# kirilllzaitsev/vision_mtl

Measured on AMD Instinct MI355X. Metric: images/sec fwd+bwd, basic model 128x256, higher is better.
Workload: dtype f32

## Files before the change

vision_mtl_amd/csrc/conv_pw.hip:

```cpp
#include "common.h"

typedef __bf16 bf16x4 __attribute__((ext_vector_type(4)));
typedef unsigned u32x4 __attribute__((ext_vector_type(4)));
__device__ __forceinline__ u32x2 pw_round_bf16x4(f32x4 v) {
  return __builtin_bit_cast(u32x2, __builtin_convertvector(v, bf16x4));
}
__device__ __forceinline__ bf16x8 pw_round_bf16x8(f32x4 lo, f32x4 hi) {
  const u32x2 l = pw_round_bf16x4(lo), h = pw_round_bf16x4(hi);
  return __builtin_bit_cast(bf16x8, (u32x4){l[0], l[1], h[0], h[1]});
}

struct PwP {
  const float* x;
  const float* wp;
  const float* bias;
  float* y;
  float* stats;
  int M, Ks, ldy, Nw, Cout;
  int tiles_m, tiles_n;
  const float* x2;
  float* y2;
  int K1, N1;
  const float* pa;
  const float* pc;
  const float* res;
  float* a_out;
  int act_in;
  const float* ez_x;
  const float* ez_mean;
  const float* ez_invstd;
  const float* ez_gamma;
  const float* ez_beta;
  const float* ez_add;
  int ez_act;
};

template <int TN, int KW, bool SRC2 = false, bool PRO = false, bool BF16 = false>
__global__ __launch_bounds__(256) void pw_gemm_kernel(PwP p) {
  constexpr int TM = 2;
  constexpr int RG = 4 / KW;
  constexpr int BM = RG * 32;
  constexpr int BN = 16 * TN;
  constexpr int OS = BN + 4;
  __shared__ __attribute__((aligned(16))) float tile[KW][BM][OS];
  __shared__ f32x4 red[2][256];

  const int tid = threadIdx.x, lane = tid & 63, wv = tid >> 6;
  const int l15 = lane & 15, lq = lane >> 4;
  const int ks = wv % KW, rg = wv / KW;
  const int bid = xcd_remap(blockIdx.x, p.tiles_m * p.tiles_n);
  const int tile_m = bid / p.tiles_n, tile_n = bid - tile_m * p.tiles_n;
  const int m0 = tile_m * BM, n0 = tile_n * BN;

  const float* ap[TM];
  const float* ap2[TM];
  const float* bp[TN];
  bool aok[TM], bok[TN];
  const int lda = SRC2 ? p.K1 : p.Ks;
#pragma unroll
  for (int i = 0; i < TM; ++i) {
    const int m = m0 + rg * 32 + 16 * i + l15;
    aok[i] = m < p.M;
    ap[i] = p.x + (size_t)(aok[i] ? m : 0) * lda + 4 * lq;
    ap2[i] = SRC2 ? p.x2 + (size_t)(aok[i] ? m : 0) * (p.Ks - p.K1) + 4 * lq - p.K1 : nullptr;
  }
#pragma unroll
  for (int j = 0; j < TN; ++j) {
    const int n = n0 + 16 * j + l15;
    bok[j] = n < p.Nw;
    bp[j] = p.wp + (size_t)(bok[j] ? n : 0) * p.Ks + 4 * lq;
  }
  const int G = (p.Ks + 15) >> 4;
  f32x4 acc[TM][TN];
#pragma unroll
  for (int i = 0; i < TM; ++i)
#pragma unroll
    for (int j = 0; j < TN; ++j) acc[i][j] = (f32x4){0.f, 0.f, 0.f, 0.f};

  struct Frag { f32x4 a[TM], b[TN], pa, pc, r[TM]; };
  auto load = [&](int g, Frag& f) {
    const bool kok = g < G && 16 * g + 4 * lq < p.Ks;
    if (PRO) {
      f.pa = kok ? *reinterpret_cast<const f32x4*>(p.pa + 16 * g + 4 * lq) : (f32x4){0.f, 0.f, 0.f, 0.f};
      f.pc = kok ? *reinterpret_cast<const f32x4*>(p.pc + 16 * g + 4 * lq) : (f32x4){0.f, 0.f, 0.f, 0.f};
    }
#pragma unroll
    for (int i = 0; i < TM; ++i) {
      const float* src = (SRC2 && 16 * g + 4 * lq >= p.K1) ? ap2[i] : ap[i];
      f.a[i] = (kok && aok[i]) ? *reinterpret_cast<const f32x4*>(src + 16 * g) : (f32x4){0.f, 0.f, 0.f, 0.f};
      if (PRO)
        f.r[i] = (p.res != nullptr && kok && aok[i]) ? *reinterpret_cast<const f32x4*>(p.res + (ap[i] - p.x) + 16 * g)
                                                     : (f32x4){0.f, 0.f, 0.f, 0.f};
    }
#pragma unroll
    for (int j = 0; j < TN; ++j)
      f.b[j] = (kok && bok[j]) ? *reinterpret_cast<const f32x4*>(bp[j] + 16 * g) : (f32x4){0.f, 0.f, 0.f, 0.f};
  };
  auto prologue = [&](Frag& f, int g) {
    if (PRO) {
#pragma unroll
      for (int i = 0; i < TM; ++i) {
        f32x4 v = f.a[i] * f.pa + f.pc;
#pragma unroll
        for (int e = 0; e < 4; ++e) v[e] = act_fwd(v[e], p.act_in);
        v += f.r[i];
        f.a[i] = v;
        if (p.a_out != nullptr && tile_n == 0 && aok[i] && g < G && 16 * g + 4 * lq < p.Ks)
          *reinterpret_cast<f32x4*>(p.a_out + (size_t)(m0 + rg * 32 + 16 * i + l15) * p.Ks + 16 * g + 4 * lq) = v;
      }
    }
  };
  auto mma = [&](Frag& f, int g) {
    prologue(f, g);
#pragma unroll
    for (int e = 0; e < 4; ++e)
#pragma unroll
      for (int i = 0; i < TM; ++i)
#pragma unroll
        for (int j = 0; j < TN; ++j)
          acc[i][j] = __builtin_amdgcn_mfma_f32_16x16x4f32(f.a[i][e], f.b[j][e], acc[i][j], 0, 0, 0);
  };
  if constexpr (!BF16) {
    Frag f0, f1, f2;
    int g = ks;
    load(g, f0);
    load(g + KW, f1);
    for (; g < G; g += 3 * KW) {
      load(g + 2 * KW, f2);
      mma(f0, g);
      if (g + KW >= G) break;
      load(g + 3 * KW, f0);
      mma(f1, g + KW);
      if (g + 2 * KW >= G) break;
      load(g + 4 * KW, f1);
      mma(f2, g + 2 * KW);
    }
  } else {
    constexpr int S = 2 * KW;
    auto load2 = [&](int g, Frag* f) {
      load(g, f[0]);
      load(g + KW, f[1]);
    };
    auto mma2 = [&](Frag* f, int g) {
      prologue(f[0], g);
      prologue(f[1], g + KW);
      bf16x8 fa[TM], fb[TN];
#pragma unroll
      for (int i = 0; i < TM; ++i) fa[i] = pw_round_bf16x8(f[0].a[i], f[1].a[i]);
#pragma unroll
      for (int j = 0; j < TN; ++j) fb[j] = pw_round_bf16x8(f[0].b[j], f[1].b[j]);
#pragma unroll
      for (int i = 0; i < TM; ++i)
#pragma unroll
        for (int j = 0; j < TN; ++j) acc[i][j] = __builtin_amdgcn_mfma_f32_16x16x32_bf16(fa[i], fb[j], acc[i][j], 0, 0, 0);
    };
    Frag f0[2], f1[2];
    int g = ks;
    load2(g, f0);
    for (; g < G; g += 2 * S) {
      load2(g + S, f1);
      mma2(f0, g);
      if (g + S >= G) break;
      load2(g + 2 * S, f0);
      mma2(f1, g + S);
    }
    (void)mma;
  }

#pragma unroll
  for (int i = 0; i < TM; ++i)
#pragma unroll
    for (int j = 0; j < TN; ++j)
#pragma unroll
      for (int r = 0; r < 4; ++r) tile[ks][rg * 32 + 16 * i + 4 * lq + r][16 * j + l15] = acc[i][j][r];
  __syncthreads();

  constexpr int Q = BN / 4;
  constexpr int RPP = 256 / Q;
  constexpr int PASSES = (BM + RPP - 1) / RPP;
  const int q = tid % Q, r0 = tid / Q;
  const int n4 = n0 + 4 * q;
  f32x4 bias4 = {0.f, 0.f, 0.f, 0.f};
  if (p.bias != nullptr) {
#pragma unroll
    for (int e = 0; e < 4; ++e)
      if (n4 + e < p.Nw) bias4[e] = p.bias[n4 + e];
  }
  f32x4 val[PASSES];
  f32x4 s1 = {0.f, 0.f, 0.f, 0.f};
  f32x4 s2x = {0.f, 0.f, 0.f, 0.f};
  const bool ez = p.ez_x != nullptr;
  f32x4 e_mean = {0.f, 0.f, 0.f, 0.f}, e_is = e_mean, e_g = e_mean, e_b = e_mean;
  if (ez && n4 < p.ldy) {
    e_mean = *reinterpret_cast<const f32x4*>(p.ez_mean + n4);
    e_is = *reinterpret_cast<const f32x4*>(p.ez_invstd + n4);
#pragma unroll
    for (int e = 0; e < 4; ++e) {
      e_g[e] = n4 + e < p.Cout ? (p.ez_gamma ? p.ez_gamma[n4 + e] : 1.f) : 0.f;
      e_b[e] = n4 + e < p.Cout ? (p.ez_beta ? p.ez_beta[n4 + e] : 0.f) : 0.f;
    }
  }
  int cnt = 0;
#pragma unroll
  for (int ps = 0; ps < PASSES; ++ps) {
    const int r = r0 + ps * RPP;
    f32x4 v = {0.f, 0.f, 0.f, 0.f};
    if (r < BM) {
      v = *reinterpret_cast<const f32x4*>(&tile[0][r][4 * q]);
#pragma unroll
      for (int k = 1; k < KW; ++k) v += *reinterpret_cast<const f32x4*>(&tile[k][r][4 * q]);
      v += bias4;
#pragma unroll
      for (int e = 0; e < 4; ++e)
        if (n4 + e >= p.Cout) v[e] = 0.f;
      const int m = m0 + r;
      if (ez && m < p.M && n4 < p.ldy) {
        if (p.ez_add != nullptr) v += *reinterpret_cast<const f32x4*>(p.ez_add + (size_t)m * p.ldy + n4);
        const f32x4 xh = (*reinterpret_cast<const f32x4*>(p.ez_x + (size_t)m * p.ldy + n4) - e_mean) * e_is;
        const f32x4 z = e_g * xh + e_b;
#pragma unroll
        for (int e = 0; e < 4; ++e) v[e] *= act_grad(z[e], p.ez_act);
        s2x += v * xh;
      }
      if (m < p.M) {
        if (n4 < p.ldy) {
          if (p.y2 == nullptr) *reinterpret_cast<f32x4*>(p.y + (size_t)m * p.ldy + n4) = v;
          else if (n4 < p.N1) *reinterpret_cast<f32x4*>(p.y + (size_t)m * p.N1 + n4) = v;
          else *reinterpret_cast<f32x4*>(p.y2 + (size_t)m * (p.ldy - p.N1) + (n4 - p.N1)) = v;
        }
        s1 += v;
        ++cnt;
      } else {
        v = (f32x4){0.f, 0.f, 0.f, 0.f};
      }
    }
    val[ps] = v;
  }
  if (p.stats != nullptr && ez) {
    red[0][tid] = s1;
    red[1][tid] = s2x;
    __syncthreads();
// ... 428 lines not shown
  if (variant == 0 && pw_big_cfg(M, ldy, Ks, &c)) {
    const int tiles_m = cdiv(M, c.bm), nprog = pw_big_nprog(M, ldy, c);
    return (M % c.bm == 0 && tiles_m % nprog == 0) ? (tiles_m / nprog) * c.bm : c.bm;
  }
  int tn, kw;
  pw_pick(M, ldy, Ks, &tn, &kw);
  return (4 / kw) * 32;
}

extern "C" int vmtl_conv1x1_stats_rows(int M, int ldy, int Ks, int variant) {
  return cdiv(M, vmtl_conv1x1_stats_block(M, ldy, Ks, variant));
}

static int pw_num_cus() {
  static int n = 0;
  if (n == 0) {
    int dev = 0;
    hipDeviceProp_t prop;
    n = (hipGetDevice(&dev) == hipSuccess && hipGetDeviceProperties(&prop, dev) == hipSuccess && prop.multiProcessorCount > 0)
            ? prop.multiProcessorCount
            : 256;
  }
  return n;
}

template <int TM, int TN, int WM, int WN, int KC, bool BF16>
static int launch_pw_big_t(PwP& p, hipStream_t st) {
  constexpr int BM = WM * TM * 16, BN = WN * TN * 16;
  constexpr int KF = BF16 ? 16 : 32;
  constexpr int A_FLOATS = KC * BM * KF, O_FLOATS = BM * (BN + 4);
  constexpr int NTHR = WM * WN * 64;
  constexpr size_t lds = ((size_t)KC * BN * KF + (A_FLOATS > O_FLOATS ? A_FLOATS : O_FLOATS)) * 4 + 2 * NTHR * 16;
  static_assert(lds <= 160 * 1024, "LDS budget");
  p.tiles_m = cdiv(p.M, BM);
  p.tiles_n = cdiv(p.ldy, BN);
  const BigCfg cfg = {0, BM, BN, KC};
  const int nprog = pw_big_nprog(p.M, p.ldy, cfg);
  const dim3 grid(nprog, p.tiles_n);
#define VMTL_PW_BIG_LAUNCH(SRC2, PRO, EZ)                                                                               \
  {                                                                                                                     \
    static bool attr_set = false;                                                                                       \
    if (!attr_set) {                                                                                                    \
      (void)hipFuncSetAttribute(reinterpret_cast<const void*>(&pw_big_kernel<TM, TN, WM, WN, KC, SRC2, PRO, EZ, BF16>), \
                                hipFuncAttributeMaxDynamicSharedMemorySize, (int)lds);                                 \
      attr_set = true;                                                                                                  \
    }                                                                                                                   \
    hipLaunchKernelGGL((pw_big_kernel<TM, TN, WM, WN, KC, SRC2, PRO, EZ, BF16>), grid, dim3(NTHR), lds, st, p, nprog);  \
  }
  if (p.ez_x != nullptr) VMTL_PW_BIG_LAUNCH(false, false, true)
  else if (p.x2 != nullptr) VMTL_PW_BIG_LAUNCH(true, false, false)
  else if (p.pa != nullptr) VMTL_PW_BIG_LAUNCH(false, true, false)
  else VMTL_PW_BIG_LAUNCH(false, false, false)
#undef VMTL_PW_BIG_LAUNCH
  return vmtl_check_launch();
}

template <int TM, int TN, int WM, int WN, int KC>
static int launch_pw_big(PwP& p, int prec, hipStream_t st) {
  return prec == VMTL_PREC_BF16 ? launch_pw_big_t<TM, TN, WM, WN, KC, true>(p, st)
                                : launch_pw_big_t<TM, TN, WM, WN, KC, false>(p, st);
}

static int pw_big_dispatch(PwP& p, const BigCfg& c, int prec, hipStream_t st) {
  static EnvInt e_w8{"VMTL_PW_BIG_WAVES", 8};
  const bool w8 = env_int(e_w8) == 8;
  switch (c.id) {
    case 0:
      if (w8)
        return c.kc == 2 ? launch_pw_big<2, 2, 2, 4, 2>(p, prec, st) : c.kc == 4 ? launch_pw_big<2, 2, 2, 4, 4>(p, prec, st)
                                                                          : launch_pw_big<2, 2, 2, 4, 6>(p, prec, st);
      return c.kc == 2 ? launch_pw_big<2, 4, 2, 2, 2>(p, prec, st) : c.kc == 4 ? launch_pw_big<2, 4, 2, 2, 4>(p, prec, st)
                                                                        : launch_pw_big<2, 4, 2, 2, 6>(p, prec, st);
    case 1:
      if (w8) return c.kc == 4 ? launch_pw_big<2, 1, 2, 4, 4>(p, prec, st) : launch_pw_big<2, 1, 2, 4, 8>(p, prec, st);
      return c.kc == 4 ? launch_pw_big<2, 2, 2, 2, 4>(p, prec, st) : launch_pw_big<2, 2, 2, 2, 8>(p, prec, st);
    case 2:
      return launch_pw_big<1, 1, 4, 2, 4>(p, prec, st);
    default:
      if (w8) return launch_pw_big<1, 3, 4, 2, 4>(p, prec, st);
      return launch_pw_big<2, 3, 2, 2, 4>(p, prec, st);
  }
}

template <int TN, int KW, bool BF16>
static int launch_pw_t(PwP& p, hipStream_t st) {
  p.tiles_m = cdiv(p.M, (4 / KW) * 32);
  p.tiles_n = cdiv(p.ldy, 16 * TN);
  if (p.x2 != nullptr)
    hipLaunchKernelGGL((pw_gemm_kernel<TN, KW, true, false, BF16>), dim3(p.tiles_m * p.tiles_n), dim3(256), 0, st, p);
  else if (p.pa != nullptr)
    hipLaunchKernelGGL((pw_gemm_kernel<TN, KW, false, true, BF16>), dim3(p.tiles_m * p.tiles_n), dim3(256), 0, st, p);
  else
    hipLaunchKernelGGL((pw_gemm_kernel<TN, KW, false, false, BF16>), dim3(p.tiles_m * p.tiles_n), dim3(256), 0, st, p);
  return vmtl_check_launch();
}

template <int TN, int KW>
static int launch_pw(PwP& p, int prec, hipStream_t st) {
  return prec == VMTL_PREC_BF16 ? launch_pw_t<TN, KW, true>(p, st) : launch_pw_t<TN, KW, false>(p, st);
}

static void pw_plain(PwP& p) {
  p.pa = p.pc = p.res = nullptr; p.a_out = nullptr; p.act_in = 0;
  p.ez_x = p.ez_mean = p.ez_invstd = p.ez_gamma = p.ez_beta = p.ez_add = nullptr; p.ez_act = 0;
}

static int pw_dispatch(PwP& p, int prec, hipStream_t st) {
  BigCfg c;
  if (p.ez_add == nullptr && p.res == nullptr && pw_big_cfg(p.M, p.ldy, p.Ks, &c)) return pw_big_dispatch(p, c, prec, st);
  int tn, kw;
  pw_pick(p.M, p.ldy, p.Ks, &tn, &kw);
  if (tn == 2) return kw == 4 ? launch_pw<2, 4>(p, prec, st) : launch_pw<2, 1>(p, prec, st);
  return kw == 4 ? launch_pw<4, 4>(p, prec, st) : launch_pw<4, 1>(p, prec, st);
}

extern "C" int vmtl_conv1x1_fwd_p(const float* x, const float* wp, const float* bias, float* y, float* stats, int M, int Ks,
                                  int ldy, int Nw, int Cout, int precision, void* stream) {
  VMTL_ENTER();
  if (!valid_prec(precision)) return VMTL_ERR_ARG;
  if (!x || !wp || !y || M <= 0 || Ks <= 0 || (Ks & 3) || ldy <= 0 || (ldy & 3)) return VMTL_ERR_ARG;
  if (Nw <= 0 || Nw > ldy || Cout <= 0 || Cout > Nw) return VMTL_ERR_ARG;
  PwP p;
  p.x = x; p.wp = wp; p.bias = bias; p.y = y; p.stats = stats; p.M = M; p.Ks = Ks; p.ldy = ldy; p.Nw = Nw; p.Cout = Cout;
  p.x2 = nullptr; p.y2 = nullptr; p.K1 = 0; p.N1 = 0;
  pw_plain(p);
  return pw_dispatch(p, precision, (hipStream_t)stream);
}

extern "C" int vmtl_conv1x1_fwd(const float* x, const float* wp, const float* bias, float* y, float* stats, int M, int Ks,
                                int ldy, int Nw, int Cout, void* stream) {
  return vmtl_conv1x1_fwd_p(x, wp, bias, y, stats, M, Ks, ldy, Nw, Cout, VMTL_PREC_FP32, stream);
}

extern "C" int vmtl_conv1x1_cat_fwd_p(const float* x, int K1, const float* x2, int K2s, const float* wp, const float* bias,
                                      float* y, float* stats, int M, int ldy, int Nw, int Cout, int precision,
                                      void* stream) {
  VMTL_ENTER();
  if (!valid_prec(precision)) return VMTL_ERR_ARG;
  if (!x || !x2 || !wp || !y || M <= 0 || K1 <= 0 || (K1 & 3) || K2s <= 0 || (K2s & 3) || ldy <= 0 || (ldy & 3))
    return VMTL_ERR_ARG;
  if (Nw <= 0 || Nw > ldy || Cout <= 0 || Cout > Nw) return VMTL_ERR_ARG;
  PwP p;
  p.x = x; p.wp = wp; p.bias = bias; p.y = y; p.stats = stats; p.M = M; p.Ks = K1 + K2s; p.ldy = ldy; p.Nw = Nw;
  p.Cout = Cout; p.x2 = x2; p.y2 = nullptr; p.K1 = K1; p.N1 = 0;
  pw_plain(p);
  return pw_dispatch(p, precision, (hipStream_t)stream);
}

extern "C" int vmtl_conv1x1_cat_fwd(const float* x, int K1, const float* x2, int K2s, const float* wp, const float* bias,
                                    float* y, float* stats, int M, int ldy, int Nw, int Cout, void* stream) {
  return vmtl_conv1x1_cat_fwd_p(x, K1, x2, K2s, wp, bias, y, stats, M, ldy, Nw, Cout, VMTL_PREC_FP32, stream);
}

extern "C" int vmtl_conv1x1_cat_dgrad_p(const float* dy, const float* wp, float* dx, int N1, float* dx2, int N2s, int N2,
                                        int M, int Ks, int precision, void* stream) {
  VMTL_ENTER();
  if (!valid_prec(precision)) return VMTL_ERR_ARG;
  if (!dy || !wp || !dx || !dx2 || M <= 0 || Ks <= 0 || (Ks & 3) || N1 <= 0 || (N1 & 3) || N2s <= 0 || (N2s & 3) ||
      N2 <= 0 || N2 > N2s)
    return VMTL_ERR_ARG;
  PwP p;
  p.x = dy; p.wp = wp; p.bias = nullptr; p.y = dx; p.stats = nullptr; p.M = M; p.Ks = Ks; p.ldy = N1 + N2s;
  p.Nw = N1 + N2; p.Cout = N1 + N2; p.x2 = nullptr; p.y2 = dx2; p.K1 = 0; p.N1 = N1;
  pw_plain(p);
  return pw_dispatch(p, precision, (hipStream_t)stream);
}

extern "C" int vmtl_conv1x1_cat_dgrad(const float* dy, const float* wp, float* dx, int N1, float* dx2, int N2s, int N2,
                                      int M, int Ks, void* stream) {
  return vmtl_conv1x1_cat_dgrad_p(dy, wp, dx, N1, dx2, N2s, N2, M, Ks, VMTL_PREC_FP32, stream);
}

static int conv1x1_bn_fwd_impl(const float* x, const float* coef_a, const float* coef_c, int act_in, const float* res,
                               float* a_out, const float* wp, const float* bias, float* y, float* stats, int M, int Ks,
                               int ldy, int Nw, int Cout, int prec, void* stream) {
  if (!x || !coef_a || !coef_c || !wp || !y || M <= 0 || Ks <= 0 || (Ks & 3) || ldy <= 0 || (ldy & 3)) return VMTL_ERR_ARG;
  if (Nw <= 0 || Nw > ldy || Cout <= 0 || Cout > Nw) return VMTL_ERR_ARG;
  if (act_in != VMTL_ACT_NONE && act_in != VMTL_ACT_RELU && act_in != VMTL_ACT_HSWISH) return VMTL_ERR_ARG;
  PwP p;
  p.x = x; p.wp = wp; p.bias = bias; p.y = y; p.stats = stats; p.M = M; p.Ks = Ks; p.ldy = ldy; p.Nw = Nw; p.Cout = Cout;
  p.x2 = nullptr; p.y2 = nullptr; p.K1 = 0; p.N1 = 0;
  pw_plain(p);
// ... 92 lines not shown
```

vision_mtl_amd/csrc/conv_wgrad.hip:

```cpp
#include <mutex>
#include <unordered_map>

#include "common.h"

struct WgradP {
  const float* x;
  const float* dy;
  float* slabs;
  int B, H, W, Cs;
  int Ho, Wo, ldy;
  int Nw;
  int KH, KW, stride, pad;
  int Ktot, M;
  int chunk;
  int tiles_kk, tiles_co, splits;
  const float* x2;
  int K1;
};

#define BP 32

typedef __bf16 bf16x2 __attribute__((ext_vector_type(2)));
typedef unsigned u32x4 __attribute__((ext_vector_type(4)));
__device__ __forceinline__ unsigned rne_bf16x2(float lo, float hi) {
  return __builtin_bit_cast(unsigned, __builtin_convertvector((f32x2){lo, hi}, bf16x2));
}
#define WG_BNK 128

__host__ __device__ constexpr int wg_ld(int w, int pm = 1) {
  return pm == 0 ? w + 4 : pm == 1 ? ((w + 47) / 64) * 64 + 16 : ((w + 15) / 32) * 32 + 16;
}
static_assert(wg_ld(16) == 16 && wg_ld(20) == 80 && wg_ld(144) == 144 && wg_ld(128) == 144 && wg_ld(68) == 80 &&
              wg_ld(80) == 80 && wg_ld(84) == 144 && wg_ld(36, 2) == 48 && wg_ld(128, 2) == 144, "wg_ld");

template <int TM, int NTR = 0, int PM = 1, int PD = (TM <= 2 ? 3 : (TM <= 4 && NTR == 0) ? 2 : 1), bool FAST = false,
          bool BF16 = false>
__global__ __launch_bounds__(256) void conv_wgrad_kernel(WgradP p) {
  constexpr int TN = 2;
  constexpr int BMM = TM * 16;
  constexpr int BMC = BMM + NTR;
  constexpr int LDY = wg_ld(BMC, PM);
  constexpr int LDX = wg_ld(WG_BNK, PM);
  constexpr int YQ = BMC / 4;
  constexpr int YIT = (BP * YQ + 255) / 256;
  constexpr int XQ = WG_BNK / 4;
  constexpr int XROWS = 256 / XQ;
  constexpr int XP = BP / XROWS;

  extern __shared__ __attribute__((aligned(16))) float smem[];
  float* Ys = smem;
  float* Xs = smem + 2 * BP * LDY;

  const int tid = threadIdx.x;
  const int lane = tid & 63, wn = tid >> 6;
  const int l15 = lane & 15, lq = lane >> 4;

  const int tiles = p.tiles_kk * p.tiles_co;
  const int bid = xcd_remap(blockIdx.x, tiles * p.splits);
  const int zsl = bid / tiles, trem = bid - zsl * tiles;
  const int kk0 = (trem % p.tiles_kk) * WG_BNK;
  const int co0 = (trem / p.tiles_kk) * BMC;
  const int p_begin = zsl * p.chunk;
  const int p_end = min(p.M, p_begin + p.chunk);

  const int xq = tid % XQ, xr = tid / XQ;
  const int kk = kk0 + xq * 4;
  const bool xok = kk < p.Ktot;
  const int tap = xok ? kk / p.Cs : 0;
  const int ci = kk - tap * p.Cs;
  const int dh = tap / p.KW - p.pad;
  const int dw = tap % p.KW - p.pad;
  const int hw = p.Ho * p.Wo;
  const bool two = p.x2 != nullptr;
  const float* xsrc = two ? (ci < p.K1 ? p.x + ci : p.x2 + (ci - p.K1)) : nullptr;
  const int xstride = two ? (ci < p.K1 ? p.K1 : p.Cs - p.K1) : 0;

  int xb[XP], xho[XP], xwo[XP];
  if (!FAST) {
#pragma unroll
    for (int i = 0; i < XP; ++i) {
      const int m = p_begin + xr + XROWS * i;
      const int b = m / hw;
      const int rem = m - b * hw;
      xb[i] = b;
      xho[i] = rem / p.Wo;
      xwo[i] = rem - xho[i] * p.Wo;
    }
  }
  int s_b = 0, s_ho = 0, s_wo = 0;
  int tw[XP];
  int toff[XP];
  int tyoff[YIT];
  if (FAST) {
    s_b = p_begin / hw;
    const int rem = p_begin - s_b * hw;
    s_ho = rem / p.Wo;
    s_wo = rem - s_ho * p.Wo;
#pragma unroll
    for (int i = 0; i < XP; ++i) {
      tw[i] = (xr + XROWS * i) * p.stride + dw;
      toff[i] = ((dh * p.W + tw[i]) * p.Cs + ci) * 4;
    }
#pragma unroll
    for (int it = 0; it < YIT; ++it) {
      const int idx = tid + it * 256;
      const int row = idx / YQ, q = idx - row * YQ;
      tyoff[it] = (idx < BP * YQ && co0 + q * 4 < p.ldy) ? (row * p.ldy + co0 + q * 4) * 4 : -1;
    }
  }

  f32x4 ry[PD][YIT], rx[PD][XP];
  const __amdgpu_buffer_rsrc_t rs_dy =
      __builtin_amdgcn_make_buffer_rsrc((void*)p.dy, 0, (int)((unsigned)p.M * p.ldy * 4u), 0x00020000);
  const __amdgpu_buffer_rsrc_t rs_x =
      __builtin_amdgcn_make_buffer_rsrc((void*)p.x, 0, (int)((unsigned)p.B * p.H * p.W * p.Cs * 4u), 0x00020000);
  constexpr unsigned OOB = 0xFFFFFFFFu;
  auto bload = [](__amdgpu_buffer_rsrc_t r, unsigned off) -> f32x4 {
    return __builtin_bit_cast(f32x4, __builtin_amdgcn_raw_buffer_load_b128(r, off, 0, 0));
  };
  auto load_tile = [&](int pp, f32x4* ry_s, f32x4* rx_s) {
    if (FAST) {
      const unsigned ybase = (unsigned)pp * (unsigned)p.ldy * 4u;
#pragma unroll
      for (int it = 0; it < YIT; ++it) ry_s[it] = bload(rs_dy, tyoff[it] >= 0 ? ybase + (unsigned)tyoff[it] : OOB);
      const int hin = s_ho * p.stride;
      const int win = s_wo * p.stride;
      const unsigned xbase = (unsigned)((s_b * p.H + hin) * p.W + win) * (unsigned)p.Cs * 4u;
      const bool hok = xok & ((unsigned)(hin + dh) < (unsigned)p.H);
#pragma unroll
      for (int i = 0; i < XP; ++i) {
        const bool ok = hok & ((unsigned)(win + tw[i]) < (unsigned)p.W);
        rx_s[i] = bload(rs_x, ok ? xbase + (unsigned)toff[i] : OOB);
      }
      s_wo += BP;
      if (s_wo >= p.Wo) {
        s_wo = 0;
        if (++s_ho == p.Ho) {
          s_ho = 0;
          ++s_b;
        }
      }
      return;
    }
#pragma unroll
    for (int it = 0; it < YIT; ++it) {
      const int idx = tid + it * 256;
      const int row = idx / YQ, q = idx - row * YQ;
      const int m = pp + row, co = co0 + q * 4;
      const bool ok = idx < BP * YQ && m < p_end && co < p.ldy;
      ry_s[it] = bload(rs_dy, ok ? ((unsigned)m * (unsigned)p.ldy + (unsigned)co) * 4u : OOB);
    }
#pragma unroll
    for (int i = 0; i < XP; ++i) {
      const int m = pp + xr + XROWS * i;
      const int h = xho[i] * p.stride + dh, w = xwo[i] * p.stride + dw;
      const bool ok = xok && m < p_end && (unsigned)h < (unsigned)p.H && (unsigned)w < (unsigned)p.W;
      const unsigned off = ((unsigned)((xb[i] * p.H + h) * p.W + w) * (unsigned)p.Cs + (unsigned)ci) * 4u;
      f32x4 v;
      if (two) {
        v = (f32x4){0.f, 0.f, 0.f, 0.f};
        if (ok) v = *reinterpret_cast<const f32x4*>(xsrc + (size_t)((xb[i] * p.H + h) * p.W + w) * xstride);
      } else {
        v = bload(rs_x, ok ? off : OOB);
      }
      rx_s[i] = v;
      xwo[i] += BP;
      while (xwo[i] >= p.Wo) {
        xwo[i] -= p.Wo;
        if (++xho[i] == p.Ho) {
          xho[i] = 0;
          ++xb[i];
        }
      }
    }
  };
  auto store_tile = [&](int buf, const f32x4* ry_s, const f32x4* rx_s) {
    float* ys = Ys + buf * BP * LDY;
    float* xs = Xs + buf * BP * LDX;
#pragma unroll
    for (int it = 0; it < YIT; ++it) {
      const int idx = tid + it * 256;
      const int row = idx / YQ, q = idx - row * YQ;
      if (idx < BP * YQ) *reinterpret_cast<f32x4*>(ys + row * LDY + q * 4) = ry_s[it];
    }
#pragma unroll
    for (int i = 0; i < XP; ++i) *reinterpret_cast<f32x4*>(xs + (xr + XROWS * i) * LDX + xq * 4) = rx_s[i];
  };

  f32x4 acc[TM][TN];
#pragma unroll
  for (int i = 0; i < TM; ++i)
#pragma unroll
    for (int j = 0; j < TN; ++j) acc[i][j] = (f32x4){0.f, 0.f, 0.f, 0.f};
  float tacc[NTR > 0 ? NTR : 1][TN];
#pragma unroll
  for (int t = 0; t < (NTR > 0 ? NTR : 1); ++t)
#pragma unroll
    for (int j = 0; j < TN; ++j) tacc[t][j] = 0.f;

  const int ntr = NTR > 0 ? max(0, min(NTR, p.Nw - (co0 + BMM))) : 0;
#pragma unroll
  for (int d = 0; d < PD; ++d)
    if (p_begin + d * BP < p_end) load_tile(p_begin + d * BP, ry[d], rx[d]);
  if (p_begin < p_end) store_tile(0, ry[0], rx[0]);
  __syncthreads();
  int cur = 0;
  const int nj = min(TN, max(0, (p.Ktot - (kk0 + wn * TN * 16) + 15) >> 4));
  auto compute = [&](int cb) {
    if (nj == 0) return;
    const float* ys = Ys + cb * BP * LDY + lq * LDY + l15;
    const float* xs = Xs + cb * BP * LDX + lq * LDX + wn * TN * 16 + l15;
    if constexpr (BF16) {
      unsigned fa[TM][4], fb[TN][4];
#pragma unroll
      for (int w = 0; w < 4; ++w) {
#pragma unroll
        for (int i = 0; i < TM; ++i)
          fa[i][w] = rne_bf16x2(ys[8 * w * LDY + i * 16], ys[(8 * w + 4) * LDY + i * 16]);
#pragma unroll
        for (int j = 0; j < TN; ++j)
          fb[j][w] = rne_bf16x2(xs[8 * w * LDX + j * 16], xs[(8 * w + 4) * LDX + j * 16]);
      }
#pragma unroll
      for (int j = 0; j < TN; ++j) {
        if (j > 0 && j >= nj) break;
        const bf16x8 b = __builtin_bit_cast(bf16x8, (u32x4){fb[j][0], fb[j][1], fb[j][2], fb[j][3]});
#pragma unroll
        for (int i = 0; i < TM; ++i)
          acc[i][j] = __builtin_amdgcn_mfma_f32_16x16x32_bf16(
              __builtin_bit_cast(bf16x8, (u32x4){fa[i][0], fa[i][1], fa[i][2], fa[i][3]}), b, acc[i][j], 0, 0, 0);
      }
      if (NTR > 0) {
#pragma unroll
        for (int s = 0; s < BP / 4; ++s) {
          const f32x4 ty = *reinterpret_cast<const f32x4*>(Ys + cb * BP * LDY + (4 * s + lq) * LDY + BMM);
#pragma unroll
          for (int t = 0; t < NTR; ++t) {
            if (t >= ntr) break;
            const float tyr = (float)(__bf16)ty[t];
#pragma unroll
            for (int j = 0; j < TN; ++j)
              tacc[t][j] += tyr * __uint_as_float((s & 1) ? (fb[j][s >> 1] & 0xFFFF0000u) : (fb[j][s >> 1] << 16));
          }
        }
      }
      return;
    }
#pragma unroll
    for (int s = 0; s < BP / 4; ++s) {
      float fa[TM], fb[TN];
#pragma unroll
      for (int i = 0; i < TM; ++i) fa[i] = ys[4 * s * LDY + i * 16];
#pragma unroll
      for (int j = 0; j < TN; ++j) fb[j] = xs[4 * s * LDX + j * 16];
#ifdef VMTL_SETPRIO
      __builtin_amdgcn_s_setprio(1);
#endif
#pragma unroll
      for (int j = 0; j < TN; ++j) {
        if (j > 0 && j >= nj) break;
#pragma unroll
        for (int i = 0; i < TM; ++i) acc[i][j] = __builtin_amdgcn_mfma_f32_16x16x4f32(fa[i], fb[j], acc[i][j], 0, 0, 0);
      }
#ifdef VMTL_SETPRIO
      __builtin_amdgcn_s_setprio(0);
#endif
      if (NTR > 0) {
        const f32x4 ty = *reinterpret_cast<const f32x4*>(Ys + cb * BP * LDY + (4 * s + lq) * LDY + BMM);
#pragma unroll
        for (int t = 0; t < NTR; ++t) {
          if (t >= ntr) break;
#pragma unroll
          for (int j = 0; j < TN; ++j) tacc[t][j] += ty[t] * fb[j];
        }
      }
    }
  };
  for (int base = p_begin; base < p_end; base += PD * BP) {
#pragma unroll
    for (int k = 0; k < PD; ++k) {
      const int pp = base + k * BP;
      if (pp < p_end) {
        if (pp + PD * BP < p_end) load_tile(pp + PD * BP, ry[k], rx[k]);
        compute(cur);
        if (pp + BP < p_end) store_tile(cur ^ 1, ry[(k + 1) % PD], rx[(k + 1) % PD]);
        __syncthreads();
        cur ^= 1;
      }
    }
  }

  float* slab = p.slabs + (size_t)zsl * p.Nw * p.Ktot;
#pragma unroll
  for (int i = 0; i < TM; ++i)
#pragma unroll
    for (int j = 0; j < TN; ++j) {
      const int col = kk0 + (wn * TN + j) * 16 + l15;
#pragma unroll
      for (int r = 0; r < 4; ++r) {
        const int row = co0 + i * 16 + 4 * lq + r;
        if (row < p.Nw && col < p.Ktot) slab[(size_t)row * p.Ktot + col] = acc[i][j][r];
      }
    }
  if (NTR > 0) {
#pragma unroll
    for (int t = 0; t < NTR; ++t)
#pragma unroll
      for (int j = 0; j < TN; ++j) {
        const float v = quarter_sum(tacc[t][j]);
        const int row = co0 + BMM + t;
        const int col = kk0 + (wn * TN + j) * 16 + l15;
        if (lq == 0 && row < p.Nw && col < p.Ktot) slab[(size_t)row * p.Ktot + col] = v;
      }
  }
}

static int wgrad_rows(int Nw) {
  static const int cands[] = {16, 32, 48, 64, 80, 144, 20, 36, 68, 128};
  static const float eff[] = {0.35f, 0.55f, 0.72f, 0.82f, 0.88f, 1.0f, 0.43f, 0.61f, 0.86f, 0.97f};
  constexpr int NC = 10;
  static EnvInt force{"VMTL_FORCE_WG_ROWS", 0};
  if (const int v = env_int(force)) {
    for (int i = 0; i < NC; ++i)
      if (cands[i] == v) return v;
  }
  int best = 16;
  float bc = -1.f;
  for (int i = 0; i < NC; ++i) {
    const float cost = (float)((long long)cdiv(Nw, cands[i]) * cands[i]) / eff[i];
    if (bc < 0.f || cost < bc) {
      best = cands[i];
      bc = cost;
    }
  }
  return best;
}

static int wgrad_lds_bytes(int rows) {
  auto lds = [&](int pm) { return 2 * BP * (wg_ld(rows, pm) + wg_ld(WG_BNK, pm)) * 4; };
  const int base = 160 * 1024 / lds(0);
  if (160 * 1024 / lds(1) >= base) return lds(1);
  if (160 * 1024 / lds(2) >= base) return lds(2);
  return lds(0);
}

static int wgrad_splits_uncached(int M, int Nw, int Ktot);

extern "C" int vmtl_conv2d_wgrad_splits(int M, int Nw, int Ktot) {
  if (M <= 0 || Nw <= 0 || Ktot <= 0) return 0;
  static std::mutex mu;
  static std::unordered_map<unsigned long long, int> memo;
  static int memo_epoch = 0;
  const unsigned long long key = ((unsigned long long)M << 32) ^ ((unsigned long long)Nw << 20) ^ (unsigned long long)Ktot;
  std::lock_guard<std::mutex> lk(mu);
  if (memo_epoch != vmtl_env_epoch) {
    memo.clear();
    memo_epoch = vmtl_env_epoch;
  }
  auto it = memo.find(key);
  if (it != memo.end()) return it->second;
  const int v = wgrad_splits_uncached(M, Nw, Ktot);
  memo.emplace(key, v);
  return v;
}

static int wgrad_splits_uncached(int M, int Nw, int Ktot) {
  const long long tiles = (long long)cdiv(Ktot, WG_BNK) * cdiv(Nw, wgrad_rows(Nw));
  static EnvInt e_steps{"VMTL_WG_MIN_STEPS", 4}, e_small{"VMTL_WG_SMALL_M", 16384}, e_splits{"VMTL_FORCE_WG_SPLITS", 0};
  const int min_steps = env_int(e_steps) < 1 ? 1 : env_int(e_steps), small_m = env_int(e_small);
  const long long max_by_rows = cdiv(M, (M <= small_m ? min_steps : 16) * BP);
  const long long max_by_mem = (32ll << 20) / ((long long)Nw * Ktot);
  long long smax = max_by_rows < max_by_mem ? max_by_rows : max_by_mem;
  if (smax < 1) smax = 1;
  if (const long long v = env_int(e_splits)) {
    if (v >= 1 && v <= max_by_rows) {
      const int chunk = cdiv(cdiv(M, (int)v), BP) * BP;
      return cdiv(M, chunk);
    }
  }
  const int rows = wgrad_rows(Nw);
  int occ = 160 * 1024 / wgrad_lds_bytes(rows);
  if (occ > 4) occ = 4;
  if (rows >= 128 && occ > 2) occ = 2;
  const long long slots = 256ll * occ;
  const double t_pix = (rows / 16.0) * occ * 0.0095;
  const double t_slab = (double)Nw * Ktot * 4.0 / 3.0e6;
  long long best = 1;
  double best_cost = -1.0;
  for (long long sp = 1; sp <= smax; ++sp) {
    const int chunk = cdiv(cdiv(M, (int)sp), BP) * BP;
    const long long nsl = cdiv(M, chunk);
    if (nsl != sp && sp != 1) continue;
    const long long rounds = cdivll(tiles * nsl, slots);
    const double cost = rounds * (chunk + 64.0) * t_pix + nsl * t_slab;
    if (best_cost < 0.0 || cost < best_cost) {
      best = nsl;
      best_cost = cost;
    }
  }
  return (int)best;
}

template <int TM, int NTR, int PM, bool FAST, bool BF16 = false>
static int launch_wgrad_pm(WgradP& p, int splits, hipStream_t st);

template <int BMC>
constexpr int wg_pm() {
  constexpr int base = 160 * 1024 / (2 * BP * (wg_ld(BMC, 0) + wg_ld(WG_BNK, 0)) * 4);
  return 160 * 1024 / (2 * BP * (wg_ld(BMC, 1) + wg_ld(WG_BNK, 1)) * 4) >= base   ? 1
         : 160 * 1024 / (2 * BP * (wg_ld(BMC, 2) + wg_ld(WG_BNK, 2)) * 4) >= base ? 2
                                                                                    : 0;
}
static_assert(wg_pm<144>() == 1 && wg_pm<80>() == 1 && wg_pm<36>() == 2 && wg_pm<68>() == 0 && wg_pm<20>() == 0 &&
                  wg_pm<128>() == 1,
              "wg_pm");

static bool wgrad_fast_ok(const WgradP& p) {
  static EnvInt e{"VMTL_WG_FAST", 1};
  return env_int(e) != 0 && p.x2 == nullptr && p.Wo % BP == 0 && p.chunk % BP == 0;
}

template <int TM, int NTR = 0>
static int launch_wgrad(WgradP& p, int splits, hipStream_t st, int prec) {
  constexpr int PMD = wg_pm<TM * 16 + NTR>();
#ifdef VMTL_TUNING
  static EnvInt e_pad{"VMTL_WG_PAD", -1};
  switch (prec == VMTL_PREC_FP32 ? env_int(e_pad) : -1) {
    case 0: return launch_wgrad_pm<TM, NTR, 0, false>(p, splits, st);
    case 1: return launch_wgrad_pm<TM, NTR, 1, false>(p, splits, st);
    case 2: return launch_wgrad_pm<TM, NTR, 2, false>(p, splits, st);
    default: break;
  }
#endif
  if (p.KH == 1 && p.KW == 1 && p.stride == 1 && p.pad == 0 && p.x2 == nullptr && p.M % BP == 0) {
    p.B = 1; p.H = 1; p.W = p.M; p.Ho = 1; p.Wo = p.M;
  }
  if (prec == VMTL_PREC_BF16) {
    if (wgrad_fast_ok(p)) return launch_wgrad_pm<TM, NTR, PMD, true, true>(p, splits, st);
    return launch_wgrad_pm<TM, NTR, PMD, false, true>(p, splits, st);
  }
  if (wgrad_fast_ok(p)) return launch_wgrad_pm<TM, NTR, PMD, true>(p, splits, st);
  return launch_wgrad_pm<TM, NTR, PMD, false>(p, splits, st);
}

template <int TM, int NTR, int PM, bool FAST, bool BF16>
static int launch_wgrad_pm(WgradP& p, int splits, hipStream_t st) {
  constexpr int BMC = TM * 16 + NTR;
  constexpr int PD = (TM <= 2 ? 3 : (TM <= 4 && NTR == 0) ? 2 : 1);
  const size_t lds = (size_t)2 * BP * (wg_ld(BMC, PM) + wg_ld(WG_BNK, PM)) * sizeof(float);
  static bool attr_set = false;
  if (!attr_set) {
    (void)hipFuncSetAttribute(reinterpret_cast<const void*>(&conv_wgrad_kernel<TM, NTR, PM, PD, FAST, BF16>),
                              hipFuncAttributeMaxDynamicSharedMemorySize, (int)lds);
    attr_set = true;
  }
  if ((long long)p.M * p.ldy * 4 >= (1ll << 32) || (long long)p.B * p.H * p.W * p.Cs * 4 >= (1ll << 32))
    return VMTL_ERR_UNSUPPORTED;
  p.tiles_kk = cdiv(p.Ktot, WG_BNK);
  p.tiles_co = cdiv(p.Nw, BMC);
  p.splits = splits;
  hipLaunchKernelGGL((conv_wgrad_kernel<TM, NTR, PM, PD, FAST, BF16>), dim3(p.tiles_kk * p.tiles_co * splits), dim3(256), lds, st,
                     p);
  return vmtl_check_launch();
}

static int wgrad_dispatch(WgradP& p, int splits, void* stream, int prec);

extern "C" int vmtl_conv2d_wgrad_p(const float* x, const float* dy, float* slabs, int splits, int B, int H, int W,
                                   int Cs, int Ho, int Wo, int ldy, int Nw, int KH, int KW, int stride, int pad,
                                   int precision, void* stream) {
  VMTL_ENTER();
  if (!valid_prec(precision) || !x || !dy || !slabs) return VMTL_ERR_ARG;
  if (Cs <= 0 || (Cs & 3) || (ldy & 3) || Nw <= 0 || Nw > ldy) return VMTL_ERR_ARG;
  if ((H + 2 * pad - KH) / stride + 1 != Ho || (W + 2 * pad - KW) / stride + 1 != Wo) return VMTL_ERR_ARG;
  if ((long long)B * Ho * Wo > 0x7fffffffLL || (long long)B * H * W > 0x7fffffffLL) return VMTL_ERR_ARG;
  WgradP p;
  p.x = x; p.dy = dy; p.slabs = slabs; p.B = B; p.H = H; p.W = W; p.Cs = Cs; p.Ho = Ho; p.Wo = Wo; p.ldy = ldy;
  p.Nw = Nw; p.KH = KH; p.KW = KW; p.stride = stride; p.pad = pad; p.Ktot = KH * KW * Cs; p.M = B * Ho * Wo;
  p.x2 = nullptr; p.K1 = 0;
  return wgrad_dispatch(p, splits, stream, precision);
}

extern "C" int vmtl_conv2d_wgrad(const float* x, const float* dy, float* slabs, int splits, int B, int H, int W,
                                 int Cs, int Ho, int Wo, int ldy, int Nw, int KH, int KW, int stride, int pad,
                                 void* stream) {
  return vmtl_conv2d_wgrad_p(x, dy, slabs, splits, B, H, W, Cs, Ho, Wo, ldy, Nw, KH, KW, stride, pad, VMTL_PREC_FP32,
                             stream);
}

extern "C" int vmtl_conv1x1_cat_wgrad_p(const float* x, int K1, const float* x2, int K2s, const float* dy, float* slabs,
                                        int splits, int M, int ldy, int Nw, int precision, void* stream) {
  VMTL_ENTER();
  if (!valid_prec(precision)) return VMTL_ERR_ARG;
  if (!x || !x2 || !dy || !slabs || M <= 0 || K1 <= 0 || (K1 & 3) || K2s <= 0 || (K2s & 3) || (ldy & 3) || Nw <= 0 ||
      Nw > ldy)
    return VMTL_ERR_ARG;
  WgradP p;
  p.x = x; p.dy = dy; p.slabs = slabs; p.B = 1; p.H = 1; p.W = M; p.Cs = K1 + K2s; p.Ho = 1; p.Wo = M; p.ldy = ldy;
  p.Nw = Nw; p.KH = 1; p.KW = 1; p.stride = 1; p.pad = 0; p.Ktot = p.Cs; p.M = M;
  p.x2 = x2; p.K1 = K1;
  return wgrad_dispatch(p, splits, stream, precision);
}

extern "C" int vmtl_conv1x1_cat_wgrad(const float* x, int K1, const float* x2, int K2s, const float* dy, float* slabs,
                                      int splits, int M, int ldy, int Nw, void* stream) {
  return vmtl_conv1x1_cat_wgrad_p(x, K1, x2, K2s, dy, slabs, splits, M, ldy, Nw, VMTL_PREC_FP32, stream);
}

static int wgrad_dispatch(WgradP& p, int splits, void* stream, int prec) {
  const int Nw = p.Nw;
  if (splits != vmtl_conv2d_wgrad_splits(p.M, Nw, p.Ktot)) return VMTL_ERR_ARG;
  p.chunk = cdiv(cdiv(p.M, splits), BP) * BP;
  hipStream_t st = (hipStream_t)stream;
  switch (wgrad_rows(Nw)) {
    case 16: return launch_wgrad<1>(p, splits, st, prec);
    case 32: return launch_wgrad<2>(p, splits, st, prec);
    case 48: return launch_wgrad<3>(p, splits, st, prec);
    case 64: return launch_wgrad<4>(p, splits, st, prec);
    case 80: return launch_wgrad<5>(p, splits, st, prec);
    case 20: return launch_wgrad<1, 4>(p, splits, st, prec);
    case 36: return launch_wgrad<2, 4>(p, splits, st, prec);
    case 68: return launch_wgrad<4, 4>(p, splits, st, prec);
    case 128: return launch_wgrad<8>(p, splits, st, prec);
    default: return launch_wgrad<9>(p, splits, st, prec);
  }
}
```

Before: 2672.

## Use buffer loads and branch-free steady-state pipelines in pointwise GEMM and wgrad

The pointwise GEMM kernel gains a PIPE path that replaces predicated global loads with raw buffer loads, using out-of-range offsets to get zero fills. Its main loop is split into a steady state with no bounds checks plus a peeled tail, and sched_barrier fences pin the load/MFMA interleave. The wgrad kernel gets a similar steady-state loop where the tail loads are masked by buffer OOB instead of being skipped by branches. Both paths are on by default behind environment switches, which increases the number of kernel instantiations and leaves the compiler less freedom in scheduling.

```diff
diff --git a/vision_mtl_amd/csrc/conv_pw.hip b/vision_mtl_amd/csrc/conv_pw.hip
--- a/vision_mtl_amd/csrc/conv_pw.hip
+++ b/vision_mtl_amd/csrc/conv_pw.hip
@@ -35,7 +35,9 @@
   int ez_act;
 };
 
-template <int TN, int KW, bool SRC2 = false, bool PRO = false, bool BF16 = false>
+__device__ __attribute__((aligned(16))) float g_pw_zero_page[4] = {0.f, 0.f, 0.f, 0.f};
+
+template <int TN, int KW, bool SRC2 = false, bool PRO = false, bool BF16 = false, bool PIPE = true>
 __global__ __launch_bounds__(256) void pw_gemm_kernel(PwP p) {
   constexpr int TM = 2;
   constexpr int RG = 4 / KW;
@@ -77,8 +79,51 @@
 #pragma unroll
     for (int j = 0; j < TN; ++j) acc[i][j] = (f32x4){0.f, 0.f, 0.f, 0.f};
 
+  unsigned aoff[TM], boff[TN];
+#pragma unroll
+  for (int i = 0; i < TM; ++i) aoff[i] = (unsigned)(ap[i] - p.x) * 4u;
+#pragma unroll
+  for (int j = 0; j < TN; ++j) boff[j] = (unsigned)(bp[j] - p.wp) * 4u;
+  constexpr unsigned OOB = 0xFFFFFFFFu;
+  const auto rsrc = [](const float* base, unsigned bytes) {
+    return __builtin_amdgcn_make_buffer_rsrc((void*)base, 0, (int)bytes, 0x00020000);
+  };
+  const __amdgpu_buffer_rsrc_t rs_a = rsrc(p.x, (unsigned)p.M * (unsigned)lda * 4u);
+  const __amdgpu_buffer_rsrc_t rs_b = rsrc(p.wp, (unsigned)p.Nw * (unsigned)p.Ks * 4u);
+  const __amdgpu_buffer_rsrc_t rs_pa = rsrc(p.pa, (unsigned)p.Ks * 4u);
+  const __amdgpu_buffer_rsrc_t rs_pc = rsrc(p.pc, (unsigned)p.Ks * 4u);
+  const __amdgpu_buffer_rsrc_t rs_res = rsrc(p.res, p.res != nullptr ? (unsigned)p.M * (unsigned)p.Ks * 4u : 0u);
+  const __amdgpu_buffer_rsrc_t rs_ao =
+      rsrc(p.a_out, (p.a_out != nullptr && tile_n == 0) ? (unsigned)p.M * (unsigned)p.Ks * 4u : 0u);
+  const auto bload = [](__amdgpu_buffer_rsrc_t r, unsigned off) -> f32x4 {
+    return __builtin_bit_cast(f32x4, __builtin_amdgcn_raw_buffer_load_b128(r, off, 0, 0));
+  };
+
   struct Frag { f32x4 a[TM], b[TN], pa, pc, r[TM]; };
   auto load = [&](int g, Frag& f) {
+    if constexpr (PIPE) {
+      const bool kok = 16 * g + 4 * lq < p.Ks;
+      const unsigned kb = 64u * (unsigned)g;
+      if (PRO) {
+        const unsigned ko = kok ? kb + 16u * (unsigned)lq : OOB;
+        f.pa = bload(rs_pa, ko);
+        f.pc = bload(rs_pc, ko);
+      }
+#pragma unroll
+      for (int i = 0; i < TM; ++i) {
+        const bool ok = kok & aok[i];
+        if (SRC2) {
+          const float* src = 16 * g + 4 * lq >= p.K1 ? ap2[i] : ap[i];
+          f.a[i] = *reinterpret_cast<const f32x4*>(ok ? src + 16 * g : g_pw_zero_page);
+        } else {
+          f.a[i] = bload(rs_a, ok ? aoff[i] + kb : OOB);
+        }
+        if (PRO) f.r[i] = bload(rs_res, ok ? aoff[i] + kb : OOB);
+      }
+#pragma unroll
+      for (int j = 0; j < TN; ++j) f.b[j] = bload(rs_b, (kok & bok[j]) ? boff[j] + kb : OOB);
+      return;
+    }
     const bool kok = g < G && 16 * g + 4 * lq < p.Ks;
     if (PRO) {
       f.pa = kok ? *reinterpret_cast<const f32x4*>(p.pa + 16 * g + 4 * lq) : (f32x4){0.f, 0.f, 0.f, 0.f};
@@ -105,7 +150,10 @@
         for (int e = 0; e < 4; ++e) v[e] = act_fwd(v[e], p.act_in);
         v += f.r[i];
         f.a[i] = v;
-        if (p.a_out != nullptr && tile_n == 0 && aok[i] && g < G && 16 * g + 4 * lq < p.Ks)
+        if constexpr (PIPE) {
+          const bool ok = aok[i] & (16 * g + 4 * lq < p.Ks);
+          __builtin_amdgcn_raw_buffer_store_b128(__builtin_bit_cast(u32x4, v), rs_ao, ok ? aoff[i] + 64u * (unsigned)g : OOB, 0, 0);
+        } else if (p.a_out != nullptr && tile_n == 0 && aok[i] && g < G && 16 * g + 4 * lq < p.Ks)
           *reinterpret_cast<f32x4*>(p.a_out + (size_t)(m0 + rg * 32 + 16 * i + l15) * p.Ks + 16 * g + 4 * lq) = v;
       }
     }
@@ -125,6 +173,27 @@
     int g = ks;
     load(g, f0);
     load(g + KW, f1);
+    if constexpr (PIPE) {
+#define FENCE() __builtin_amdgcn_sched_barrier(0)
+      for (; g + 4 * KW < G; g += 3 * KW) {
+        load(g + 2 * KW, f2); FENCE();
+        mma(f0, g); FENCE();
+        load(g + 3 * KW, f0); FENCE();
+        mma(f1, g + KW); FENCE();
+        load(g + 4 * KW, f1); FENCE();
+        mma(f2, g + 2 * KW); FENCE();
+      }
+      load(g + 2 * KW, f2); FENCE();
+      if (g < G) mma(f0, g);
+      FENCE();
+      load(g + 3 * KW, f0); FENCE();
+      if (g + KW < G) mma(f1, g + KW);
+      FENCE();
+      if (g + 2 * KW < G) mma(f2, g + 2 * KW);
+      FENCE();
+      if (g + 3 * KW < G) mma(f0, g + 3 * KW);
+      g = G;
+    }
     for (; g < G; g += 3 * KW) {
       load(g + 2 * KW, f2);
       mma(f0, g);
@@ -157,6 +226,23 @@
     Frag f0[2], f1[2];
     int g = ks;
     load2(g, f0);
+    if constexpr (PIPE) {
+      for (; g + 2 * S + KW < G; g += 2 * S) {
+        load2(g + S, f1); FENCE();
+        mma2(f0, g); FENCE();
+        load2(g + 2 * S, f0); FENCE();
+        mma2(f1, g + S); FENCE();
+      }
+      load2(g + S, f1); FENCE();
+      if (g < G) mma2(f0, g);
+      FENCE();
+      load2(g + 2 * S, f0); FENCE();
+      if (g + S < G) mma2(f1, g + S);
+      FENCE();
+      if (g + 2 * S < G) mma2(f0, g + 2 * S);
+#undef FENCE
+      g = G;
+    }
     for (; g < G; g += 2 * S) {
       load2(g + S, f1);
       mma2(f0, g);
@@ -751,22 +837,33 @@
   }
 }
 
-template <int TN, int KW, bool BF16>
+static bool pw_pipe_ok(const PwP& p) {
+  static EnvInt e{"VMTL_PW_PIPE", 1};
+  if (!env_int(e)) return false;
+  const unsigned long long lim = 1ull << 32;
+  const unsigned long long lda = p.x2 != nullptr ? p.K1 : p.Ks;
+  return (unsigned long long)p.M * lda * 4 < lim && (unsigned long long)p.Nw * p.Ks * 4 < lim &&
+         (unsigned long long)p.M * p.Ks * 4 < lim;
+}
+
+template <int TN, int KW, bool BF16, bool PIPE>
 static int launch_pw_t(PwP& p, hipStream_t st) {
   p.tiles_m = cdiv(p.M, (4 / KW) * 32);
   p.tiles_n = cdiv(p.ldy, 16 * TN);
   if (p.x2 != nullptr)
-    hipLaunchKernelGGL((pw_gemm_kernel<TN, KW, true, false, BF16>), dim3(p.tiles_m * p.tiles_n), dim3(256), 0, st, p);
+    hipLaunchKernelGGL((pw_gemm_kernel<TN, KW, true, false, BF16, PIPE>), dim3(p.tiles_m * p.tiles_n), dim3(256), 0, st, p);
   else if (p.pa != nullptr)
-    hipLaunchKernelGGL((pw_gemm_kernel<TN, KW, false, true, BF16>), dim3(p.tiles_m * p.tiles_n), dim3(256), 0, st, p);
+    hipLaunchKernelGGL((pw_gemm_kernel<TN, KW, false, true, BF16, PIPE>), dim3(p.tiles_m * p.tiles_n), dim3(256), 0, st, p);
   else
-    hipLaunchKernelGGL((pw_gemm_kernel<TN, KW, false, false, BF16>), dim3(p.tiles_m * p.tiles_n), dim3(256), 0, st, p);
+    hipLaunchKernelGGL((pw_gemm_kernel<TN, KW, false, false, BF16, PIPE>), dim3(p.tiles_m * p.tiles_n), dim3(256), 0, st, p);
   return vmtl_check_launch();
 }
 
 template <int TN, int KW>
 static int launch_pw(PwP& p, int prec, hipStream_t st) {
-  return prec == VMTL_PREC_BF16 ? launch_pw_t<TN, KW, true>(p, st) : launch_pw_t<TN, KW, false>(p, st);
+  if (pw_pipe_ok(p))
+    return prec == VMTL_PREC_BF16 ? launch_pw_t<TN, KW, true, true>(p, st) : launch_pw_t<TN, KW, false, true>(p, st);
+  return prec == VMTL_PREC_BF16 ? launch_pw_t<TN, KW, true, false>(p, st) : launch_pw_t<TN, KW, false, false>(p, st);
 }
 
 static void pw_plain(PwP& p) {
diff --git a/vision_mtl_amd/csrc/conv_wgrad.hip b/vision_mtl_amd/csrc/conv_wgrad.hip
--- a/vision_mtl_amd/csrc/conv_wgrad.hip
+++ b/vision_mtl_amd/csrc/conv_wgrad.hip
@@ -34,7 +34,7 @@
               wg_ld(80) == 80 && wg_ld(84) == 144 && wg_ld(36, 2) == 48 && wg_ld(128, 2) == 144, "wg_ld");
 
 template <int TM, int NTR = 0, int PM = 1, int PD = (TM <= 2 ? 3 : (TM <= 4 && NTR == 0) ? 2 : 1), bool FAST = false,
-          bool BF16 = false>
+          bool BF16 = false, bool PIPE = false>
 __global__ __launch_bounds__(256) void conv_wgrad_kernel(WgradP p) {
   constexpr int TN = 2;
   constexpr int BMM = TM * 16;
@@ -118,15 +118,16 @@
   auto bload = [](__amdgpu_buffer_rsrc_t r, unsigned off) -> f32x4 {
     return __builtin_bit_cast(f32x4, __builtin_amdgcn_raw_buffer_load_b128(r, off, 0, 0));
   };
-  auto load_tile = [&](int pp, f32x4* ry_s, f32x4* rx_s) {
+  auto load_tile = [&](int pp, f32x4* ry_s, f32x4* rx_s, bool live = true) {
     if (FAST) {
       const unsigned ybase = (unsigned)pp * (unsigned)p.ldy * 4u;
 #pragma unroll
-      for (int it = 0; it < YIT; ++it) ry_s[it] = bload(rs_dy, tyoff[it] >= 0 ? ybase + (unsigned)tyoff[it] : OOB);
+      for (int it = 0; it < YIT; ++it)
+        ry_s[it] = bload(rs_dy, ((tyoff[it] >= 0) & live) ? ybase + (unsigned)tyoff[it] : OOB);
       const int hin = s_ho * p.stride;
       const int win = s_wo * p.stride;
       const unsigned xbase = (unsigned)((s_b * p.H + hin) * p.W + win) * (unsigned)p.Cs * 4u;
-      const bool hok = xok & ((unsigned)(hin + dh) < (unsigned)p.H);
+      const bool hok = xok & live & ((unsigned)(hin + dh) < (unsigned)p.H);
 #pragma unroll
       for (int i = 0; i < XP; ++i) {
         const bool ok = hok & ((unsigned)(win + tw[i]) < (unsigned)p.W);
@@ -200,8 +201,10 @@
 
   const int ntr = NTR > 0 ? max(0, min(NTR, p.Nw - (co0 + BMM))) : 0;
 #pragma unroll
-  for (int d = 0; d < PD; ++d)
-    if (p_begin + d * BP < p_end) load_tile(p_begin + d * BP, ry[d], rx[d]);
+  for (int d = 0; d < PD; ++d) {
+    if constexpr (PIPE) load_tile(p_begin + d * BP, ry[d], rx[d], p_begin + d * BP < p_end);
+    else if (p_begin + d * BP < p_end) load_tile(p_begin + d * BP, ry[d], rx[d]);
+  }
   if (p_begin < p_end) store_tile(0, ry[0], rx[0]);
   __syncthreads();
   int cur = 0;
@@ -276,12 +279,26 @@
       }
     }
   };
-  for (int base = p_begin; base < p_end; base += PD * BP) {
+  int base = p_begin;
+  if constexpr (PIPE) {
+    for (; base + (2 * PD - 1) * BP < p_end; base += PD * BP) {
+#pragma unroll
+      for (int k = 0; k < PD; ++k) {
+        load_tile(base + (k + PD) * BP, ry[k], rx[k]);
+        compute(cur);
+        store_tile(cur ^ 1, ry[(k + 1) % PD], rx[(k + 1) % PD]);
+        __syncthreads();
+        cur ^= 1;
+      }
+    }
+  }
+  for (; base < p_end; base += PD * BP) {
 #pragma unroll
     for (int k = 0; k < PD; ++k) {
       const int pp = base + k * BP;
       if (pp < p_end) {
-        if (pp + PD * BP < p_end) load_tile(pp + PD * BP, ry[k], rx[k]);
+        if constexpr (PIPE) load_tile(pp + PD * BP, ry[k], rx[k], pp + PD * BP < p_end);
+        else if (pp + PD * BP < p_end) load_tile(pp + PD * BP, ry[k], rx[k]);
         compute(cur);
         if (pp + BP < p_end) store_tile(cur ^ 1, ry[(k + 1) % PD], rx[(k + 1) % PD]);
         __syncthreads();
@@ -443,14 +460,27 @@
   return launch_wgrad_pm<TM, NTR, PMD, false>(p, splits, st);
 }
 
+template <int TM, int NTR, int PM, bool FAST, bool BF16, bool PIPE>
+static int launch_wgrad_pipe(WgradP& p, int splits, hipStream_t st);
+
 template <int TM, int NTR, int PM, bool FAST, bool BF16>
 static int launch_wgrad_pm(WgradP& p, int splits, hipStream_t st) {
+  constexpr int PD = (TM <= 2 ? 3 : (TM <= 4 && NTR == 0) ? 2 : 1);
+  if constexpr (PD >= 3 && FAST) {
+    static EnvInt e{"VMTL_WG_PIPE", 1};
+    if (env_int(e)) return launch_wgrad_pipe<TM, NTR, PM, FAST, BF16, true>(p, splits, st);
+  }
+  return launch_wgrad_pipe<TM, NTR, PM, FAST, BF16, false>(p, splits, st);
+}
+
+template <int TM, int NTR, int PM, bool FAST, bool BF16, bool PIPE>
+static int launch_wgrad_pipe(WgradP& p, int splits, hipStream_t st) {
   constexpr int BMC = TM * 16 + NTR;
   constexpr int PD = (TM <= 2 ? 3 : (TM <= 4 && NTR == 0) ? 2 : 1);
   const size_t lds = (size_t)2 * BP * (wg_ld(BMC, PM) + wg_ld(WG_BNK, PM)) * sizeof(float);
   static bool attr_set = false;
   if (!attr_set) {
-    (void)hipFuncSetAttribute(reinterpret_cast<const void*>(&conv_wgrad_kernel<TM, NTR, PM, PD, FAST, BF16>),
+    (void)hipFuncSetAttribute(reinterpret_cast<const void*>(&conv_wgrad_kernel<TM, NTR, PM, PD, FAST, BF16, PIPE>),
                               hipFuncAttributeMaxDynamicSharedMemorySize, (int)lds);
     attr_set = true;
   }
@@ -459,7 +489,7 @@
   p.tiles_kk = cdiv(p.Ktot, WG_BNK);
   p.tiles_co = cdiv(p.Nw, BMC);
   p.splits = splits;
-  hipLaunchKernelGGL((conv_wgrad_kernel<TM, NTR, PM, PD, FAST, BF16>), dim3(p.tiles_kk * p.tiles_co * splits), dim3(256), lds, st,
+  hipLaunchKernelGGL((conv_wgrad_kernel<TM, NTR, PM, PD, FAST, BF16, PIPE>), dim3(p.tiles_kk * p.tiles_co * splits), dim3(256), lds, st,
                      p);
   return vmtl_check_launch();
 }
```

Measured after the change: 2717 (median of 6 runs). 1.7% higher.
